# pudnax/voidin

Measured on AMD Instinct MI355X. Metric: M instances culled+compacted/sec, higher is better.
Workload: dtype f32; 1 GPU; configs[2]: 10M synthetic AABB instances, cull + prefix-sum compaction (BASELINE.md §3 distribution, model.rs camera); instances_per_gpu=10000000, instances_total=10000000, n_meshes=16, distribution=baseline, parallelism=single GPU

## Files before the change

### voidin_amd/csrc/cull.hip

```cpp
#include "vd_common.hpp"

#include <math.h>

namespace {

constexpr int kWave = 64;
constexpr int kBlock = 256;
constexpr int kWavesPerBlock = kBlock / kWave;
constexpr int kInstBytes = 144;
constexpr int kSlabBytes = kWave * kInstBytes;
constexpr int kChunksPerLane = kSlabBytes / (kWave * 16);



typedef unsigned int u32x4 __attribute__((ext_vector_type(4)));

struct CullCamera {
    float view[16];
    float frustum[4];
    float znear, zfar;
};

struct MeshRec { float mnx, mny, mnz; unsigned index_count; float mxx, mxy, mxz; unsigned base_index; int vertex_offset; };

// ... 561 lines not shown
    const float d = -c[2];
    const float dn = d - r;
    if (!(dn > znear)) return false;
    const float rr = r * r, dd = d * d, rd = r * d;
    const float tx = sqrtf((c[0] * c[0] + dd) - rr), ty = sqrtf((c[1] * c[1] + dd) - rr);
    const float dxm = d * tx + c[0] * r, dxp = d * tx - c[0] * r, dym = d * ty + c[1] * r, dyp = d * ty - c[1] * r;
    if (!(dxm > 0.0f && dxp > 0.0f && dym > 0.0f && dyp > 0.0f)) return false;
    const float sx0 = (c[0] * tx - rd) / dxm, sx1 = (c[0] * tx + rd) / dxp;
    const float sy0 = (c[1] * ty - rd) / dym, sy1 = (c[1] * ty + rd) / dyp;
    const float nxa = P.p00 * sx0 - P.p20, nxb = P.p00 * sx1 - P.p20, nya = P.p11 * sy0 - P.p21, nyb = P.p11 * sy1 - P.p21;
    const float nx_lo = fminf(nxa, nxb), nx_hi = fmaxf(nxa, nxb), ny_lo = fminf(nya, nyb), ny_hi = fmaxf(nya, nyb);
    const float W = (float)hz.width, H = (float)hz.height;
    const float u0 = (nx_lo * 0.5f + 0.5f) * W - 0.5f, u1 = (nx_hi * 0.5f + 0.5f) * W + 0.5f;
    const float v0 = (0.5f - ny_hi * 0.5f) * H - 0.5f, v1 = (0.5f - ny_lo * 0.5f) * H + 0.5f;
    if (!(u1 >= 0.0f && v1 >= 0.0f && u0 < W && v0 < H)) return false;
    const unsigned x0 = (unsigned)floorf(fmaxf(u0, 0.0f)), x1 = (unsigned)floorf(fminf(u1, W - 1.0f));
    const unsigned y0 = (unsigned)floorf(fmaxf(v0, 0.0f)), y1 = (unsigned)floorf(fminf(v1, H - 1.0f));
    const unsigned span = max(x1 - x0, y1 - y0);
    const unsigned lvl = min(span ? 32u - (unsigned)__clz((int)span) : 0u, hz.n_levels - 1u);
    const float* t = hz.base + hz.off[lvl];
    const unsigned lw = ((hz.width - 1u) >> lvl) + 1u;
    const unsigned ax = x0 >> lvl, bx = x1 >> lvl, ay = y0 >> lvl, by = y1 >> lvl;
    const float h0 = fminf(t[(size_t)ay * lw + ax], t[(size_t)ay * lw + bx]);
    const float h1 = fminf(t[(size_t)by * lw + ax], t[(size_t)by * lw + bx]);
    const float hmin = fminf(h0, h1);
    const float depth = (P.p32 - P.p22 * dn) / dn;
    return depth < hmin;
}

template <typename IdT, bool HIZ, bool PREV>
__global__ __launch_bounds__(kBlock, 3) void cull_mask_occ_kernel(CullCamera cam, OccProj proj, HizView hz, const VdMeshInfo* __restrict__ meshes,
                                                                   unsigned n_mesh, const VdInstance* __restrict__ inst, unsigned n_inst,
                                                                   vd_u64* __restrict__ mask, const vd_u64* prev, vd_u64* visible_out,
                                                                   IdT* __restrict__ ids_out, unsigned* __restrict__ tile_count,
                                                                   unsigned n_tiles) {
    extern __shared__ __attribute__((aligned(16))) char smem[];
    const unsigned lane = threadIdx.x & 63u, wave = threadIdx.x >> 6;
    constexpr int kIdBytes = TileIds<IdT>::kBytes;
    char* slab = smem + wave * (kSlabBytes + kIdBytes);
    IdT* s_ids = reinterpret_cast<IdT*>(slab + kSlabBytes);
    const unsigned waves_total = gridDim.x * kWavesPerBlock;
    const size_t n_words = ((size_t)n_inst + 63) / 64;
    auto valid_at = [&](size_t f) -> unsigned { return f < n_inst ? (unsigned)min((size_t)64, (size_t)n_inst - f) : 0u; };
    u32x4 regs[kChunksPerLane];
    for (unsigned t = blockIdx.x * kWavesPerBlock + wave; t < n_tiles; t += waves_total) {
        const size_t tile_first = (size_t)t * (kWave * kMaskRounds);
        const size_t w0 = (size_t)t * kMaskRounds;
        const bool my_slot = lane < (unsigned)kMaskRounds && w0 + lane < n_words;
        slab_fill<true>(inst, tile_first, valid_at(tile_first), lane, regs);
        unsigned p_lo = 0u, p_hi = 0u;
        if (PREV && my_slot) { const vd_u64 p = prev[w0 + lane]; p_lo = (unsigned)p; p_hi = (unsigned)(p >> 32); }
        TileIds<IdT> tile_ids;
        tile_ids.load(ids_out, tile_first, n_inst, lane);
        vd_u64 list_word = 0, vis_word = 0;
#pragma unroll 1
        for (int r = 0; r < kMaskRounds; ++r) {
            const size_t first = tile_first + (size_t)r * kWave;
            const unsigned n_valid = valid_at(first);
            slab_store(slab, lane, regs);
            if (r + 1 < kMaskRounds) slab_fill<true>(inst, first + kWave, valid_at(first + kWave), lane, regs);
            vd_wave_lds_sync();
            const LaneInst li = slab_read(slab, lane);
            vd_wave_lds_sync();
            const unsigned mid = min(li.mesh, n_mesh - 1u);
            const MeshRec m = load_mesh(meshes, mid);
            const ViewCentre vc = view_centre(cam.view, m, li.T0, li.T1, li.T2, li.T3);
            bool keep = lane < n_valid && frustum_visible(cam, m, vc);
            if (HIZ) {
                if (__ballot(keep) != 0ull) {
                    if (keep) keep = !sphere_occluded(proj, cam.znear, hz, m, vc);
                }
            }
            vd_u64 b = __ballot(keep);
            if (PREV) {
                const vd_u64 p = (vd_u64)(unsigned)__builtin_amdgcn_readlane((int)p_lo, r) |
                                 ((vd_u64)(unsigned)__builtin_amdgcn_readlane((int)p_hi, r) << 32);
                if (HIZ) { if (lane == (unsigned)r) vis_word = b; b &= ~p; }
                else b &= p;
            }
            if (lane == (unsigned)r) list_word = b;
            s_ids[r * kWave + lane] = (IdT)mid;
        }
        vd_wave_lds_sync();
        if (my_slot) {
            mask[w0 + lane] = list_word;
            if (HIZ && PREV) visible_out[w0 + lane] = vis_word;
        }
        unsigned survivors = (unsigned)__popcll(list_word);
#pragma unroll
        for (int off = kMaskRounds / 2; off > 0; off >>= 1) survivors += __shfl_xor(survivors, off);
        if (lane == 0u) tile_count[t] = survivors;
        tile_ids.flush(ids_out, s_ids, tile_first, n_inst, lane);
        vd_wave_lds_sync();
    }
}

constexpr int kExpandGroup = 4;
constexpr int kExpandWords = 32;
constexpr int kChunkWords = kWavesPerBlock * kExpandWords;

constexpr int kScanBlock = 1024;
struct ScanState { unsigned done, epoch, pad[2]; };
__global__ __launch_bounds__(kScanBlock) void mask_scan_kernel(const vd_u64* __restrict__ mask, unsigned n_words, unsigned n_chunks,
                                                           vd_u64* chunk_entry, ScanState* state,
                                                           unsigned* __restrict__ out_count) {
    constexpr int kScanWaves = kScanBlock / kWave;
    __shared__ unsigned s_last, s_wave_sum[kScanWaves];
    const unsigned lane = threadIdx.x & 63u, wave = threadIdx.x >> 6;
    const unsigned ep = __hip_atomic_load(&state->epoch, VD_RLX_AGENT);
    const vd_u64 tag = (vd_u64)ep << 32;
    for (unsigned c = blockIdx.x * kScanWaves + wave; c < n_chunks; c += gridDim.x * kScanWaves) {
        const unsigned w = c * kChunkWords + lane;
        unsigned v = (w < n_words ? (unsigned)__popcll(mask[w]) : 0u) + (w + 64u < n_words ? (unsigned)__popcll(mask[w + 64u]) : 0u);
#pragma unroll
        for (int off = 32; off > 0; off >>= 1) v += __shfl_xor(v, off);
        if (lane == 0) __hip_atomic_store(&chunk_entry[c], tag | v, VD_RLX_AGENT);
    }
    __builtin_amdgcn_s_waitcnt(0);
    __syncthreads();
    if (threadIdx.x == 0) s_last = __hip_atomic_fetch_add(&state->done, 1u, VD_RLX_AGENT) == gridDim.x - 1u;
    __syncthreads();
    if (!s_last) return;
    const unsigned per = (n_chunks + kScanBlock - 1) / kScanBlock;
    const unsigned begin = min(threadIdx.x * per, n_chunks), end = min(begin + per, n_chunks);
    bool stuck = false;
    auto entry = [&](unsigned c) -> unsigned {
        vd_u64 e = __hip_atomic_load(&chunk_entry[c], VD_RLX_AGENT);
        unsigned spins = 0;
        while ((e >> 32) != (vd_u64)ep) {
            if (++spins > (1u << 22)) { stuck = true; return 0u; }
            __builtin_amdgcn_s_sleep(1);
            e = __hip_atomic_load(&chunk_entry[c], VD_RLX_AGENT);
        }
        return (unsigned)e;
    };
    unsigned sum = 0;
    for (unsigned c = begin; c < end; ++c) sum += entry(c);
    const bool any_stuck = __syncthreads_or(stuck ? 1 : 0) != 0;
    unsigned incl = sum;
#pragma unroll
    for (int off = 1; off < kWave; off <<= 1) {
        const unsigned t = __shfl_up(incl, off);
        if (lane >= (unsigned)off) incl += t;
    }
    if (lane == kWave - 1u) s_wave_sum[wave] = incl;
    __syncthreads();
    unsigned run = incl - sum;
    for (unsigned w = 0; w < wave; ++w) run += s_wave_sum[w];
    for (unsigned c = begin; c < end; ++c) {
        if (any_stuck) { chunk_entry[c] = tag | 0xffffffffu; continue; }
        const unsigned v = entry(c);
        chunk_entry[c] = tag | run;
        run += v;
    }
    if (threadIdx.x == kScanBlock - 1u) {
        *out_count = any_stuck ? 0xffffffffu : run;
        __hip_atomic_store(&state->done, 0u, VD_RLX_AGENT);
        __hip_atomic_store(&state->epoch, ep + 1u, VD_RLX_AGENT);
    }
}

constexpr int kChunkTiles = kChunkWords / kMaskRounds;

__device__ __forceinline__ unsigned tile_prefix_partial(const unsigned* __restrict__ tile_count, unsigned n_before) {
    constexpr unsigned kBatch = 4;
    unsigned sum = 0;
    for (unsigned i0 = threadIdx.x * 4u; i0 < n_before; i0 += kBatch * kBlock * 4u) {
        u32x4 v[kBatch];
#pragma unroll
        for (unsigned k = 0; k < kBatch; ++k) {
            const unsigned i = i0 + k * kBlock * 4u;
            v[k] = *reinterpret_cast<const u32x4*>(tile_count + (i < n_before ? i : i0));
        }
#pragma unroll
        for (unsigned k = 0; k < kBatch; ++k) {
            const unsigned i = i0 + k * kBlock * 4u;
            sum += (i < n_before ? v[k].x : 0u) + (i + 1u < n_before ? v[k].y : 0u) + (i + 2u < n_before ? v[k].z : 0u) +
                   (i + 3u < n_before ? v[k].w : 0u);
        }
    }
#pragma unroll
    for (int off = 32; off > 0; off >>= 1) sum += __shfl_xor(sum, off);
    return sum;
}

template <typename IdT, bool TAB, bool TILES>
__global__ __launch_bounds__(kBlock) void expand_mask_kernel(const vd_u64* __restrict__ mask, unsigned n_words, unsigned wps,
                                                             unsigned shard_size, unsigned n_total, unsigned first_instance,
                                                             const IdT* __restrict__ mesh_ids,
                                                             const VdMeshInfo* __restrict__ meshes, unsigned n_mesh,
                                                             VdDrawIndexedIndirect* __restrict__ out,
                                                             const vd_u64* __restrict__ chunk_entry,
                                                             const unsigned* __restrict__ tile_count, unsigned* __restrict__ out_count) {
    constexpr int kGroups = kExpandWords / kExpandGroup;
    __shared__ unsigned s_prefix[kWavesPerBlock];
    constexpr unsigned kTab = TAB ? 512 : 1;
    __shared__ unsigned s_tab[kTab][3];
    constexpr int kStageBytes = kExpandGroup * 1280 + 32;
    __shared__ __attribute__((aligned(16))) char s_stage[kWavesPerBlock][kStageBytes];
    const unsigned lane = threadIdx.x & 63u, wave = threadIdx.x >> 6;
    const unsigned chunk = blockIdx.x;
    const unsigned cw0 = chunk * kChunkWords;
    const unsigned w0 = __builtin_amdgcn_readfirstlane(cw0 + wave * kExpandWords);
    unsigned base = 0;
    if (TILES) {
        const unsigned part = tile_prefix_partial(tile_count, chunk * kChunkTiles);
        if (lane == 0) s_prefix[wave] = part;
    } else {
        base = (unsigned)chunk_entry[chunk];
        if (base == 0xffffffffu) return;
    }
    unsigned before = 0;
    if (lane < wave * kExpandWords && cw0 + lane < n_words) before = (unsigned)__popcll(mask[cw0 + lane]);
    if (lane + 64u < wave * kExpandWords && cw0 + 64u + lane < n_words) before += (unsigned)__popcll(mask[cw0 + 64u + lane]);
    vd_u64 my_word = 0;
    if (lane < (unsigned)kExpandWords && w0 + lane < n_words) my_word = mask[w0 + lane];
    auto group_first = [&](unsigned wg, unsigned (&f)[kExpandGroup]) {
        unsigned shard = wg / wps, r = wg - shard * wps;
#pragma unroll
        for (int q = 0; q < kExpandGroup; ++q) {
            f[q] = shard * shard_size + 64u * r;
            if (++r >= wps) { r = 0u; ++shard; }
        }
    };
    unsigned ids[kExpandWords];
#pragma unroll
    for (int g = 0; g < kGroups; ++g) {
        const unsigned wg = w0 + g * kExpandGroup;
        unsigned f[kExpandGroup];
        group_first(wg, f);
#pragma unroll
        for (int q = 0; q < kExpandGroup; ++q) {
            const unsigned idx = f[q] + lane;
            ids[g * kExpandGroup + q] = (wg + q < n_words && idx < n_total) ? (unsigned)mesh_ids[idx] : 0u;
        }
    }
    if (TAB)
        for (unsigned i = threadIdx.x; i < n_mesh; i += kBlock) {
            s_tab[i][0] = meshes[i].index_count; s_tab[i][1] = meshes[i].base_index; s_tab[i][2] = (unsigned)meshes[i].vertex_offset;
        }
#pragma unroll
    for (int off = 32; off > 0; off >>= 1) before += __shfl_xor(before, off);
    base += before;
    __syncthreads();
    if (TILES) {
#pragma unroll
        for (int w = 0; w < kWavesPerBlock; ++w) base += s_prefix[w];
        if (chunk == gridDim.x - 1u && wave == kWavesPerBlock - 1u) {
            unsigned mine = (unsigned)__popcll(my_word);
#pragma unroll
            for (int off = 32; off > 0; off >>= 1) mine += __shfl_xor(mine, off);
            if (lane == 0) *out_count = base + mine;
        }
    }
    char* stage = s_stage[wave];
#pragma unroll
    for (int g = 0; g < kGroups; ++g) {
        const unsigned wg = w0 + g * kExpandGroup;
        vd_u64 m[kExpandGroup];
        unsigned cnt = 0;
#pragma unroll
        for (int q = 0; q < kExpandGroup; ++q) {
            const int k = g * kExpandGroup + q;
            const unsigned lo = __shfl((unsigned)my_word, k), hi = __shfl((unsigned)(my_word >> 32), k);
            m[q] = ((vd_u64)hi << 32) | lo;
            cnt += (unsigned)__popcll(m[q]);
        }
        if (cnt == 0u) continue;
        char* gbase = reinterpret_cast<char*>(out + base);
        const unsigned shift = (unsigned)(reinterpret_cast<uintptr_t>(gbase) & 15u);
        unsigned run = 0;
        unsigned first[kExpandGroup];
        group_first(wg, first);
#pragma unroll
        for (int q = 0; q < kExpandGroup; ++q) {
            unsigned mid = ids[g * kExpandGroup + q];
            if ((m[q] >> lane) & 1ull) {
                mid = min(mid, n_mesh - 1u);
                unsigned* o = reinterpret_cast<unsigned*>(stage + shift + 20u * (run + vd_mbcnt(m[q])));
                if (TAB) { o[0] = s_tab[mid][0]; o[2] = s_tab[mid][1]; o[3] = s_tab[mid][2]; }
                else { o[0] = meshes[mid].index_count; o[2] = meshes[mid].base_index; o[3] = (unsigned)meshes[mid].vertex_offset; }
                o[1] = 1u;
                o[4] = first_instance + first[q] + lane;
            }
            run += (unsigned)__popcll(m[q]);
        }
        vd_wave_lds_sync();
        const unsigned total = shift + 20u * cnt;
        char* g16 = gbase - shift;
        for (unsigned b0 = lane * 16u; b0 < total; b0 += kWave * 16u) {
            if (b0 >= shift && b0 + 16u <= total) {
                *reinterpret_cast<u32x4*>(g16 + b0) = *reinterpret_cast<const u32x4*>(stage + b0);
            } else {
                const unsigned lo_b = b0 > shift ? b0 : shift, hi_b = b0 + 16u < total ? b0 + 16u : total;
                for (unsigned b = lo_b; b < hi_b; b += 4u)
                    *reinterpret_cast<unsigned*>(g16 + b) = *reinterpret_cast<const unsigned*>(stage + b);
            }
        }
        vd_wave_lds_sync();
        base += cnt;
    }
}

template <bool DIRECT, bool TILES>
__global__ __launch_bounds__(kBlock) void expand_mask_u8_kernel(const vd_u64* __restrict__ mask, unsigned n_words, unsigned wps,
                                                                unsigned shard_size, unsigned n_total, unsigned first_instance,
                                                                const unsigned char* __restrict__ mesh_ids,
                                                                const VdMeshInfo* __restrict__ meshes, unsigned n_mesh,
                                                                VdDrawIndexedIndirect* __restrict__ out,
                                                                const vd_u64* __restrict__ chunk_entry,
                                                                const unsigned* __restrict__ tile_count, unsigned* __restrict__ out_count) {
    constexpr int kGroups = kExpandWords / kExpandGroup;
    __shared__ unsigned s_prefix[kWavesPerBlock];
    __shared__ __attribute__((aligned(16))) unsigned s_tab[256][4];
    constexpr int kStageBytes = DIRECT ? 16 : kExpandGroup * 1280 + 32;
    __shared__ __attribute__((aligned(16))) char s_stage[kWavesPerBlock][kStageBytes];
    const unsigned lane = threadIdx.x & 63u;
    const unsigned wave = __builtin_amdgcn_readfirstlane(threadIdx.x >> 6);
    const unsigned chunk = blockIdx.x;
    const unsigned cw0 = chunk * kChunkWords;
    const unsigned w0 = cw0 + wave * kExpandWords;
    unsigned base = 0;
    if (TILES) {
        const unsigned part = tile_prefix_partial(tile_count, chunk * kChunkTiles);
        if (lane == 0) s_prefix[wave] = part;
    } else {
        base = (unsigned)chunk_entry[chunk];
        if (base == 0xffffffffu) return;
    }
    unsigned before = 0;
    if (lane < wave * kExpandWords && cw0 + lane < n_words) before = (unsigned)__popcll(mask[cw0 + lane]);
    if (lane + 64u < wave * kExpandWords && cw0 + 64u + lane < n_words) before += (unsigned)__popcll(mask[cw0 + 64u + lane]);
    vd_u64 my_word = 0;
    if (lane < (unsigned)kExpandWords && w0 + lane < n_words) my_word = mask[w0 + lane];
    unsigned ids[kGroups];
    {
        const unsigned wl = w0 + (lane >> 4);
        unsigned shard = wl / wps, r = wl - shard * wps;
#pragma unroll
        for (int g = 0; g < kGroups; ++g) {
            const unsigned i0 = shard * shard_size + 64u * r + 4u * (lane & 15u);
            ids[g] = (wl + g * kExpandGroup < n_words && i0 < n_total) ? *reinterpret_cast<const unsigned*>(mesh_ids + i0) : 0u;
            r += kExpandGroup;
            if (r >= wps) { r -= wps; ++shard; }
        }
    }
    unsigned s_shard = w0 / wps, s_r = w0 - s_shard * wps;
    unsigned word_first = s_shard * shard_size + 64u * s_r;
    constexpr unsigned PF = DIRECT ? 0u : 32u;
    unsigned pf = 0;
    if (PF > 0) {
        const unsigned pw = (chunk + 8u * PF) * kChunkWords + (threadIdx.x >> 1);
        if (pw < n_words) {
            const unsigned ps = pw / wps;
            const unsigned pi = ps * shard_size + 64u * (pw - ps * wps) + 32u * (threadIdx.x & 1u);
            if (pi + 32u <= n_total) {
                const u32x4 a = *reinterpret_cast<const u32x4*>(mesh_ids + pi), b = *reinterpret_cast<const u32x4*>(mesh_ids + pi + 16u);
                pf = a.x ^ a.w ^ b.x ^ b.w;
            }
            if ((threadIdx.x & 1u) == 0u) pf ^= (unsigned)mask[pw];
        }
    }
    if (threadIdx.x < n_mesh) {
        const VdMeshInfo mi = meshes[threadIdx.x];
        s_tab[threadIdx.x][0] = mi.index_count; s_tab[threadIdx.x][1] = 1u;
        s_tab[threadIdx.x][2] = mi.base_index;  s_tab[threadIdx.x][3] = (unsigned)mi.vertex_offset;
    }
#pragma unroll
    for (int off = 32; off > 0; off >>= 1) before += __shfl_xor(before, off);
    base = __builtin_amdgcn_readfirstlane(base + before);
    __syncthreads();
    if (TILES) {
#pragma unroll
        for (int w = 0; w < kWavesPerBlock; ++w) base += s_prefix[w];
        base = __builtin_amdgcn_readfirstlane(base);
        if (chunk == gridDim.x - 1u && wave == kWavesPerBlock - 1u) {
            unsigned mine = (unsigned)__popcll(my_word);
#pragma unroll
            for (int off = 32; off > 0; off >>= 1) mine += __shfl_xor(mine, off);
            if (lane == 0) *out_count = base + mine;
        }
    }
    const unsigned max_mid = n_mesh - 1u;
    const unsigned inst_lane = first_instance + lane;
    const unsigned id_shift = 8u * (lane & 3u);
    char* stage = s_stage[wave];
#pragma unroll
    for (int g = 0; g < kGroups; ++g) {
        vd_u64 m[kExpandGroup];
        unsigned cnt = 0;
#pragma unroll
        for (int q = 0; q < kExpandGroup; ++q) {
            const int k = g * kExpandGroup + q;
            const unsigned lo = __builtin_amdgcn_readlane((unsigned)my_word, k), hi = __builtin_amdgcn_readlane((unsigned)(my_word >> 32), k);
            m[q] = ((vd_u64)hi << 32) | lo;
            cnt += (unsigned)__popcll(m[q]);
        }
        unsigned wf[kExpandGroup];
#pragma unroll
        for (int q = 0; q < kExpandGroup; ++q) {
            wf[q] = word_first;
            if (++s_r >= wps) { s_r = 0u; ++s_shard; }
            word_first = s_shard * shard_size + 64u * s_r;
        }
        if (cnt == 0u) continue;
        if (DIRECT) {
            unsigned run = base;
#pragma unroll
            for (int q = 0; q < kExpandGroup; ++q) {
                const unsigned v = (unsigned)__shfl((int)ids[g], q * 16 + (int)(lane >> 2));
                const unsigned mid = min((v >> id_shift) & 0xffu, max_mid);
                if (__builtin_amdgcn_inverse_ballot_w64(m[q])) {
                    unsigned* o = reinterpret_cast<unsigned*>(out + (run + vd_mbcnt(m[q])));
                    typedef u32x4 __attribute__((aligned(4))) u32x4_a4;
                    *reinterpret_cast<u32x4_a4*>(o) = *reinterpret_cast<const u32x4*>(s_tab[mid]);
                    o[4] = inst_lane + wf[q];
                }
                run += (unsigned)__popcll(m[q]);
            }
        } else {
            char* gbase = reinterpret_cast<char*>(out + base);
            const unsigned shift = (unsigned)(reinterpret_cast<uintptr_t>(gbase) & 15u);
            unsigned run = 0;
#pragma unroll
            for (int q = 0; q < kExpandGroup; ++q) {
                const unsigned v = (unsigned)__shfl((int)ids[g], q * 16 + (int)(lane >> 2));
                const unsigned mid = min((v >> id_shift) & 0xffu, max_mid);
                if (__builtin_amdgcn_inverse_ballot_w64(m[q])) {
                    unsigned* o = reinterpret_cast<unsigned*>(stage + shift + 20u * (run + vd_mbcnt(m[q])));
                    const u32x4 c = *reinterpret_cast<const u32x4*>(s_tab[mid]);
                    o[0] = c.x; o[1] = c.y; o[2] = c.z; o[3] = c.w;
                    o[4] = inst_lane + wf[q];
                }
                run += (unsigned)__popcll(m[q]);
            }
            vd_wave_lds_sync();
            const unsigned total = shift + 20u * cnt;
            char* g16 = gbase - shift;
            for (unsigned b0 = lane * 16u; b0 < total; b0 += kWave * 16u) {
                if (b0 >= shift && b0 + 16u <= total) {
                    *reinterpret_cast<u32x4*>(g16 + b0) = *reinterpret_cast<const u32x4*>(stage + b0);
                } else {
                    const unsigned lo_b = b0 > shift ? b0 : shift, hi_b = b0 + 16u < total ? b0 + 16u : total;
                    for (unsigned b = lo_b; b < hi_b; b += 4u)
                        *reinterpret_cast<unsigned*>(g16 + b) = *reinterpret_cast<const unsigned*>(stage + b);
                }
            }
            vd_wave_lds_sync();
        }
        base += cnt;
    }
    if (PF > 0 && pf == 0x9e3779b9u && n_mesh == 0u) out[0].instance_count = pf;
}

template <typename IdT>
__global__ __launch_bounds__(kBlock) void emit_from_mask_kernel(const vd_u64* __restrict__ mask, const IdT* __restrict__ mesh_ids,
                                                               const VdMeshInfo* __restrict__ meshes, unsigned n_mesh,
                                                               unsigned n_inst, unsigned first_instance,
                                                               VdDrawIndexedIndirect* __restrict__ out) {
    constexpr unsigned kTab = 512;
    __shared__ __attribute__((aligned(16))) unsigned s_tab[kTab][4];
    const bool tab = n_mesh <= kTab;
    if (tab)
        for (unsigned i = threadIdx.x; i < n_mesh; i += kBlock) {
            s_tab[i][0] = meshes[i].index_count; s_tab[i][1] = 0u;
            s_tab[i][2] = meshes[i].base_index;  s_tab[i][3] = (unsigned)meshes[i].vertex_offset;
        }
    __syncthreads();
    const unsigned n_quads = (n_inst + 3u) / 4u;
    for (unsigned q = blockIdx.x * kBlock + threadIdx.x; q < n_quads; q += gridDim.x * kBlock) {
        const unsigned i0 = q * 4u;
        const unsigned bits = (unsigned)(mask[i0 >> 6] >> (i0 & 63u)) & 15u;
        unsigned mid[4];
#pragma unroll
        for (int k = 0; k < 4; ++k) mid[k] = i0 + k < n_inst ? min((unsigned)mesh_ids[i0 + k], n_mesh - 1u) : 0u;
        unsigned w[20];
#pragma unroll
        for (int k = 0; k < 4; ++k) {
            u32x4 c;
            if (tab) c = *reinterpret_cast<const u32x4*>(s_tab[mid[k]]);
            else { c.x = meshes[mid[k]].index_count; c.z = meshes[mid[k]].base_index; c.w = (unsigned)meshes[mid[k]].vertex_offset; }
            w[5 * k] = c.x; w[5 * k + 1] = (bits >> k) & 1u; w[5 * k + 2] = c.z; w[5 * k + 3] = c.w; w[5 * k + 4] = first_instance + i0 + k;
        }
        unsigned* o = reinterpret_cast<unsigned*>(out + i0);
        if (i0 + 4u <= n_inst) {
#pragma unroll
            for (int k = 0; k < 5; ++k) {
                u32x4 v; v.x = w[4 * k]; v.y = w[4 * k + 1]; v.z = w[4 * k + 2]; v.w = w[4 * k + 3];
                *reinterpret_cast<u32x4*>(o + 4 * k) = v;
            }
        } else {
            for (unsigned k = 0; k < 5u * (n_inst - i0); ++k) o[k] = w[k];
        }
    }
}

__global__ __launch_bounds__(kBlock) void emit_all_u8_kernel(const vd_u64* __restrict__ mask, unsigned n_words, unsigned n_inst,
                                                             unsigned first_instance, const unsigned char* __restrict__ mesh_ids,
                                                             const VdMeshInfo* __restrict__ meshes, unsigned n_mesh,
                                                             VdDrawIndexedIndirect* __restrict__ out) {
    constexpr int kGroups = kExpandWords / kExpandGroup;
    __shared__ __attribute__((aligned(16))) unsigned s_tab[256][4];
    const unsigned lane = threadIdx.x & 63u;
    const unsigned wave = __builtin_amdgcn_readfirstlane(threadIdx.x >> 6);
    const unsigned w0 = (blockIdx.x * kWavesPerBlock + wave) * kExpandWords;
    vd_u64 my_word = 0;
    if (lane < (unsigned)kExpandWords && w0 + lane < n_words) my_word = mask[w0 + lane];
    unsigned ids[kGroups];
#pragma unroll
    for (int g = 0; g < kGroups; ++g) {
        const unsigned i0 = 64u * (w0 + g * kExpandGroup + (lane >> 4)) + 4u * (lane & 15u);
        ids[g] = i0 < n_inst ? *reinterpret_cast<const unsigned*>(mesh_ids + i0) : 0u;
    }
    if (threadIdx.x < n_mesh) {
        const VdMeshInfo mi = meshes[threadIdx.x];
        s_tab[threadIdx.x][0] = mi.index_count; s_tab[threadIdx.x][1] = 0u;
        s_tab[threadIdx.x][2] = mi.base_index;  s_tab[threadIdx.x][3] = (unsigned)mi.vertex_offset;
    }
    __syncthreads();
    const unsigned max_mid = n_mesh - 1u;
    const unsigned id_shift = 8u * (lane & 3u);
#pragma unroll
    for (int g = 0; g < kGroups; ++g) {
#pragma unroll
        for (int q = 0; q < kExpandGroup; ++q) {
            const int k = g * kExpandGroup + q;
            const unsigned lo = __builtin_amdgcn_readlane((unsigned)my_word, k), hi = __builtin_amdgcn_readlane((unsigned)(my_word >> 32), k);
            const vd_u64 m = ((vd_u64)hi << 32) | lo;
            const unsigned v = (unsigned)__shfl((int)ids[g], q * 16 + (int)(lane >> 2));
            const unsigned mid = min((v >> id_shift) & 0xffu, max_mid);
            const unsigned i = 64u * (w0 + (unsigned)k) + lane;
            if (i < n_inst) {
                u32x4 c = *reinterpret_cast<const u32x4*>(s_tab[mid]);
                c.y = (unsigned)(m >> lane) & 1u;
                unsigned* o = reinterpret_cast<unsigned*>(out + i);
                typedef u32x4 __attribute__((aligned(4))) u32x4_a4;
                *reinterpret_cast<u32x4_a4*>(o) = c;
                o[4] = first_instance + i;
            }
        }
    }
}

__global__ __launch_bounds__(kBlock) void mask_to_indices_kernel(const vd_u64* __restrict__ mask, unsigned n_words, unsigned first_instance,
                                                                 unsigned* __restrict__ out, const vd_u64* __restrict__ chunk_entry) {
    const unsigned lane = threadIdx.x & 63u;
    const unsigned wave = __builtin_amdgcn_readfirstlane(threadIdx.x >> 6);
    const unsigned cw0 = blockIdx.x * kChunkWords;
    const unsigned w0 = cw0 + wave * kExpandWords;
    unsigned base = (unsigned)chunk_entry[blockIdx.x];
    if (base == 0xffffffffu) return;
    unsigned before = 0;
    if (lane < wave * kExpandWords && cw0 + lane < n_words) before = (unsigned)__popcll(mask[cw0 + lane]);
    if (lane + 64u < wave * kExpandWords && cw0 + 64u + lane < n_words) before += (unsigned)__popcll(mask[cw0 + 64u + lane]);
    vd_u64 my_word = 0;
    if (lane < (unsigned)kExpandWords && w0 + lane < n_words) my_word = mask[w0 + lane];
#pragma unroll
    for (int off = 32; off > 0; off >>= 1) before += __shfl_xor(before, off);
    base = __builtin_amdgcn_readfirstlane(base + before);
    const unsigned inst_lane = first_instance + 64u * w0 + lane;
#pragma unroll
    for (int k = 0; k < kExpandWords; ++k) {
        const unsigned lo = __builtin_amdgcn_readlane((unsigned)my_word, k), hi = __builtin_amdgcn_readlane((unsigned)(my_word >> 32), k);
        const vd_u64 m = ((vd_u64)hi << 32) | lo;
        if (__builtin_amdgcn_inverse_ballot_w64(m)) out[base + vd_mbcnt(m)] = inst_lane + 64u * (unsigned)k;
        base += (unsigned)__popcll(m);
    }
}

template <typename IdT>
__global__ __launch_bounds__(kBlock) void indices_to_draws_kernel(const unsigned* __restrict__ indices, unsigned n_indices,
                                                                  const IdT* __restrict__ mesh_ids, unsigned n_total,
                                                                  const VdMeshInfo* __restrict__ meshes, unsigned n_mesh,
                                                                  VdDrawIndexedIndirect* __restrict__ out) {
    constexpr unsigned kTab = 512;
    __shared__ __attribute__((aligned(16))) unsigned s_tab[kTab][4];
    const bool tab = n_mesh <= kTab;
    if (tab)
        for (unsigned i = threadIdx.x; i < n_mesh; i += kBlock) {
            s_tab[i][0] = meshes[i].index_count; s_tab[i][1] = 1u;
            s_tab[i][2] = meshes[i].base_index;  s_tab[i][3] = (unsigned)meshes[i].vertex_offset;
        }
    __syncthreads();
    for (unsigned k = blockIdx.x * kBlock + threadIdx.x; k < n_indices; k += gridDim.x * kBlock) {
        const unsigned i = indices[k];
        const unsigned mid = min((unsigned)mesh_ids[min(i, n_total - 1u)], n_mesh - 1u);
        u32x4 c;
        if (tab) c = *reinterpret_cast<const u32x4*>(s_tab[mid]);
        else { c.x = meshes[mid].index_count; c.y = 1u; c.z = meshes[mid].base_index; c.w = (unsigned)meshes[mid].vertex_offset; }
        unsigned* o = reinterpret_cast<unsigned*>(out + k);
        typedef u32x4 __attribute__((aligned(4))) u32x4_a4;
        *reinterpret_cast<u32x4_a4*>(o) = c;
        o[4] = i;
    }
}

static int launch_mask_scan(VdCtx* ctx, const vd_u64* d_mask, unsigned n_words, unsigned* d_out_count, vd_u64** out_entries) {
    const unsigned n_chunks = (n_words + kChunkWords - 1) / kChunkWords;
    const size_t need = sizeof(ScanState) + (size_t)n_chunks * 8;
    if (need > ctx->expand_state_bytes || !ctx->expand_state) {
        int rc = vd_ensure(ctx, &ctx->expand_state, &ctx->expand_state_bytes, need);
        if (rc) return rc;
        VD_HIP_CHECK(ctx, hipMemsetAsync(ctx->expand_state, 0, ctx->expand_state_bytes, ctx->stream));
        VD_HIP_CHECK(ctx, hipMemsetD32Async(reinterpret_cast<hipDeviceptr_t>(reinterpret_cast<char*>(ctx->expand_state) + offsetof(ScanState, epoch)), 1, 1, ctx->stream));
    }
    ScanState* state = reinterpret_cast<ScanState*>(ctx->expand_state);
    vd_u64* entries = reinterpret_cast<vd_u64*>(reinterpret_cast<char*>(ctx->expand_state) + sizeof(ScanState));
    unsigned sblocks = (n_chunks + 15u) / 16u;
    if (sblocks > (unsigned)ctx->num_cus * 2u) sblocks = (unsigned)ctx->num_cus * 2u;
    hipLaunchKernelGGL(mask_scan_kernel, dim3(sblocks), dim3(kScanBlock), 0, ctx->stream, d_mask, n_words, n_chunks, entries, state,
                       d_out_count);
    *out_entries = entries;
    return VD_OK;
}

static int launch_expand(VdCtx* ctx, const vd_u64* d_mask, unsigned n_words, unsigned wps, unsigned shard_size,
                         unsigned n_total, unsigned first_instance, const void* d_ids, unsigned id_bytes,
                         const VdMeshInfo* d_meshes, unsigned n_mesh, VdDrawIndexedIndirect* d_out, unsigned* d_out_count,
                         const unsigned* d_tile_count = nullptr) {
    const unsigned n_chunks = (n_words + kChunkWords - 1) / kChunkWords;
    vd_u64* offsets = nullptr;
    if (!d_tile_count) {
        int rc_scan = launch_mask_scan(ctx, d_mask, n_words, d_out_count, &offsets);
        if (rc_scan) return rc_scan;
    }
    const bool one_shard = wps >= n_words;
    const bool tab = n_mesh <= 512u;
    const bool fast = id_bytes == 1u && n_mesh <= 256u && (one_shard || (shard_size % 4u == 0u && wps >= (unsigned)kExpandGroup)) &&
                      (reinterpret_cast<uintptr_t>(d_ids) & 3u) == 0u;
    if (fast) {
#define VD_EXPAND_U8(D, T)                                                                                                  \
        hipLaunchKernelGGL((expand_mask_u8_kernel<D, T>), dim3(n_chunks), dim3(kBlock), 0, ctx->stream, d_mask, n_words, wps, \
                           shard_size, n_total, first_instance, reinterpret_cast<const unsigned char*>(d_ids), d_meshes,      \
                           n_mesh, d_out, offsets, d_tile_count, d_out_count)
        const bool direct = n_total <= (12u << 20);
        if (d_tile_count) { if (direct) VD_EXPAND_U8(true, true); else VD_EXPAND_U8(false, true); }
        else { if (direct) VD_EXPAND_U8(true, false); else VD_EXPAND_U8(false, false); }
#undef VD_EXPAND_U8
        return VD_OK;
    }
#define VD_EXPAND_T(IdT, T, S)                                                                                             \
    hipLaunchKernelGGL((expand_mask_kernel<IdT, T, S>), dim3(n_chunks), dim3(kBlock), 0, ctx->stream, d_mask, n_words, wps, \
                       shard_size, n_total, first_instance, reinterpret_cast<const IdT*>(d_ids), d_meshes, n_mesh, d_out,    \
                       offsets, d_tile_count, d_out_count)
#define VD_EXPAND(IdT, T) do { if (d_tile_count) VD_EXPAND_T(IdT, T, true); else VD_EXPAND_T(IdT, T, false); } while (0)
    if (id_bytes == 1u) { if (tab) VD_EXPAND(unsigned char, true); else VD_EXPAND(unsigned char, false); }
    else if (id_bytes == 2u) { if (tab) VD_EXPAND(unsigned short, true); else VD_EXPAND(unsigned short, false); }
    else { if (tab) VD_EXPAND(unsigned, true); else VD_EXPAND(unsigned, false); }
#undef VD_EXPAND
#undef VD_EXPAND_T
    return VD_OK;
}

__global__ __launch_bounds__(kBlock) void pad_tail_kernel(VdDrawIndexedIndirect* __restrict__ out,
                                                          const unsigned* __restrict__ count, unsigned n) {
    const unsigned c = *count;
    const size_t begin = (c > n ? (size_t)0 : (size_t)c) * 5u, end = (size_t)n * 5u;
    unsigned* o = reinterpret_cast<unsigned*>(out);
    if (begin >= end) return;
    const size_t gid = (size_t)blockIdx.x * kBlock + threadIdx.x, gsz = (size_t)gridDim.x * kBlock;
    const size_t mis = (reinterpret_cast<uintptr_t>(o + begin) >> 2) & 3u;
    const size_t head = min(end - begin, (4u - mis) & 3u);
    const size_t quads = (end - begin - head) >> 2;
    const size_t tail_first = begin + head + quads * 4u;
    if (gid < head) o[begin + gid] = 0u;
    if (gid < end - tail_first) o[tail_first + gid] = 0u;
    u32x4* q = reinterpret_cast<u32x4*>(o + begin + head);
    const u32x4 z = {0u, 0u, 0u, 0u};
    for (size_t i = gid; i < quads; i += gsz) __builtin_nontemporal_store(z, q + i);
}

constexpr int kCompactPerThread = 8;
constexpr int kCompactTile = kBlock * kCompactPerThread;

__global__ __launch_bounds__(kBlock) void compact_draws_kernel(const VdDrawIndexedIndirect* __restrict__ in, unsigned n,
                                                               VdDrawIndexedIndirect* __restrict__ out,
                                                               unsigned* __restrict__ out_count, vd_u64* tile_state,
                                                               vd_u64* ticket_counter, unsigned n_tiles, unsigned* fault_host) {
    __shared__ unsigned s_ticket, s_epoch, s_wave_total[kWavesPerBlock], s_tile_excl;
    const unsigned lane = threadIdx.x & 63u, wave = threadIdx.x >> 6;
    if (threadIdx.x == 0) s_ticket = vd_take_ticket(ticket_counter, n_tiles, &s_epoch);
    __syncthreads();
    const unsigned tile = s_ticket, epoch = s_epoch;
    if (tile >= n_tiles) return;
    if (tile == 0u && threadIdx.x == 0) { __hip_atomic_store(out_count, VD_SCAN_STUCK, VD_RLX_AGENT); __threadfence(); }
    const size_t wave_first = (size_t)tile * kCompactTile + (size_t)wave * (kWave * kCompactPerThread);
    unsigned long long masks[kCompactPerThread];
    unsigned wave_total = 0;
    const unsigned* in32 = reinterpret_cast<const unsigned*>(in);
#pragma unroll
    for (int r = 0; r < kCompactPerThread; ++r) {
        const size_t i = wave_first + (size_t)r * kWave + lane;
        const bool keep = i < n && in32[i * 5u + 1u] == 1u;
        masks[r] = __ballot(keep);
        wave_total += (unsigned)__popcll(masks[r]);
    }
    if (lane == 0) s_wave_total[wave] = wave_total;
    __syncthreads();
    if (wave == 0) {
        unsigned tile_total = 0;
#pragma unroll
        for (int w = 0; w < kWavesPerBlock; ++w) tile_total += s_wave_total[w];
        const unsigned excl = vd_lookback(tile_state, epoch, tile, tile_total);
        if (lane == 0) {
            s_tile_excl = excl;
            if (tile == n_tiles - 1u) *out_count = vd_scan_final_count(tile_state, epoch, excl, tile_total, fault_host);
        }
    }
    __syncthreads();
    unsigned base = s_tile_excl;
    if (base == VD_SCAN_STUCK) return;
    for (unsigned w = 0; w < wave; ++w) base += s_wave_total[w];
    unsigned* out32 = reinterpret_cast<unsigned*>(out);
#pragma unroll
    for (int r = 0; r < kCompactPerThread; ++r) {
        const unsigned long long mask = masks[r];
        if ((mask >> lane) & 1ull) {
            const size_t i = wave_first + (size_t)r * kWave + lane;
            const size_t d = (size_t)(base + vd_mbcnt(mask)) * 5u;
#pragma unroll
            for (int k = 0; k < 5; ++k) out32[d + k] = in32[i * 5u + k];
        }
        base += (unsigned)__popcll(mask);
    }
}

struct RotZ { float c_pos, s_pos, c_neg, s_neg; };
template <int SRC> __device__ __forceinline__ float quad_bcast(float v) {
    return __int_as_float(__builtin_amdgcn_mov_dpp(__float_as_int(v), SRC * 0x55, 0xf, 0xf, true));
}
__global__ __launch_bounds__(256) void compute_update_kernel(const unsigned* __restrict__ indices, unsigned n_indices,
                                                             VdInstance* __restrict__ inst, unsigned n_inst, RotZ rz, int fix_inverse) {
    const unsigned t = blockIdx.x * 256u + threadIdx.x, k = t >> 2, col = t & 3u;
    const unsigned idx = k < n_indices ? indices[k] : 0xffffffffu;
    const bool live = idx < n_inst;
    float4* t4 = reinterpret_cast<float4*>(inst[live ? idx : 0u].transform);
    float4 v = make_float4(0.0f, 0.0f, 0.0f, 0.0f);
    if (live) v = t4[col];
    const float t14 = quad_bcast<3>(v.z);
    const bool pos = t14 > -15.0f;
    const float c = pos ? rz.c_pos : rz.c_neg, s = pos ? rz.s_pos : rz.s_neg;
    float4 o;
    o.x = ((c * v.x + -s * v.y) + 0.0f * v.z) + 0.0f * v.w;
    o.y = ((s * v.x + c * v.y) + 0.0f * v.z) + 0.0f * v.w;
    o.z = ((0.0f * v.x + 0.0f * v.y) + 1.0f * v.z) + 0.0f * v.w;
    o.w = ((0.0f * v.x + 0.0f * v.y) + 0.0f * v.z) + 1.0f * v.w;
    if (live) t4[col] = o;
    if (fix_inverse) {
        float4* i4 = reinterpret_cast<float4*>(inst[live ? idx : 0u].inv_transform);
        float4 w = make_float4(0.0f, 0.0f, 0.0f, 0.0f);
        if (live) w = i4[col];
        const float4 I0 = make_float4(quad_bcast<0>(w.x), quad_bcast<0>(w.y), quad_bcast<0>(w.z), quad_bcast<0>(w.w));
        const float4 I1 = make_float4(quad_bcast<1>(w.x), quad_bcast<1>(w.y), quad_bcast<1>(w.z), quad_bcast<1>(w.w));
        const float4 I2 = make_float4(quad_bcast<2>(w.x), quad_bcast<2>(w.y), quad_bcast<2>(w.z), quad_bcast<2>(w.w));
        const float4 I3 = make_float4(quad_bcast<3>(w.x), quad_bcast<3>(w.y), quad_bcast<3>(w.z), quad_bcast<3>(w.w));
        const float b0 = col == 0u ? c : (col == 1u ? s : 0.0f);
        const float b1 = col == 0u ? -s : (col == 1u ? c : 0.0f);
        const float b2 = col == 2u ? 1.0f : 0.0f, b3 = col == 3u ? 1.0f : 0.0f;
        float4 r;
        r.x = ((I0.x * b0 + I1.x * b1) + I2.x * b2) + I3.x * b3;
        r.y = ((I0.y * b0 + I1.y * b1) + I2.y * b2) + I3.y * b3;
        r.z = ((I0.z * b0 + I1.z * b1) + I2.z * b2) + I3.z * b3;
        r.w = ((I0.w * b0 + I1.w * b1) + I2.w * b2) + I3.w * b3;
        if (live) i4[col] = r;
    }
}

CullCamera make_cam(const VdCameraUniform* c) {
    CullCamera k;
    memcpy(k.view, c->view, sizeof(k.view));
    memcpy(k.frustum, c->frustum, sizeof(k.frustum));
    k.znear = c->znear;
    k.zfar = c->zfar;
    return k;
}

}

extern "C" {

int vd_cull_emit_dev(VdCtx* ctx, const VdCameraUniform* camera, const VdMeshInfo* d_meshes, uint32_t n_mesh,
                     const VdInstance* d_instances, uint32_t n_inst, VdDrawIndexedIndirect* d_out) {
    VdDeviceGuard vd_guard_(ctx);
    return vd_cull_emit_shard_dev(ctx, camera, d_meshes, n_mesh, d_instances, n_inst, 0u, d_out);
}

static int launch_mask_pass(VdCtx* ctx, const VdCameraUniform* camera, const VdMeshInfo* d_meshes, uint32_t n_mesh,
                            const VdInstance* d_instances, uint32_t n_inst, vd_u64** out_mask, void** out_ids, unsigned* out_id_bytes,
                            unsigned** out_tile_count) {
    const unsigned n_words = (n_inst + 63u) / 64u;
    const unsigned id_bytes = n_mesh <= 256u ? 1u : (n_mesh <= 65536u ? 2u : 4u);
    const unsigned n_mt = (n_inst + kWave * kMaskRounds - 1) / (kWave * kMaskRounds);
    const size_t ids_off = ((size_t)n_words * 8 + 255) & ~(size_t)255;
    const size_t counts_off = (ids_off + (size_t)n_inst * id_bytes + 15) & ~(size_t)15;
    const size_t need = counts_off + (((size_t)n_mt + 3) & ~(size_t)3) * 4 + 512;
    int rc = vd_ensure(ctx, &ctx->scratch, &ctx->scratch_bytes, need);
    if (rc) return rc;
    vd_u64* d_mask = reinterpret_cast<vd_u64*>(ctx->scratch);
    void* d_ids = reinterpret_cast<char*>(ctx->scratch) + ids_off;
    unsigned* d_counts = reinterpret_cast<unsigned*>(reinterpret_cast<char*>(ctx->scratch) + counts_off);
    vd_time_begin(ctx);
    unsigned mb = (n_mt + kWavesPerBlock - 1) / kWavesPerBlock;
    if (mb > (unsigned)ctx->num_cus * 3u) mb = (unsigned)ctx->num_cus * 3u;
#define VD_SPLIT(IdT)                                                                                              \
    hipLaunchKernelGGL(cull_mask_tiled_kernel<IdT>, dim3(mb), dim3(kBlock),                                        \
                       kWavesPerBlock * (kSlabBytes + kMaskRounds * kWave * (int)sizeof(IdT)),                     \
                       ctx->stream, make_cam(camera), d_meshes, n_mesh, d_instances, n_inst, d_mask,               \
                       reinterpret_cast<IdT*>(d_ids), d_counts, n_mt)
    if (id_bytes == 1u) VD_SPLIT(unsigned char);
    else if (id_bytes == 2u) VD_SPLIT(unsigned short);
    else VD_SPLIT(unsigned);
#undef VD_SPLIT
    vd_time_mid(ctx);
    *out_mask = d_mask; *out_ids = d_ids; *out_id_bytes = id_bytes; *out_tile_count = d_counts;
    return VD_OK;
}

int vd_cull_emit_shard_dev(VdCtx* ctx, const VdCameraUniform* camera, const VdMeshInfo* d_meshes, uint32_t n_mesh,
                           const VdInstance* d_instances, uint32_t n_inst, uint32_t first_instance,
                           VdDrawIndexedIndirect* d_out) {
    VdDeviceGuard vd_guard_(ctx);
    if (!ctx) return VD_ERR_INVALID_ARG;
    if (!camera || !d_meshes || n_mesh == 0) VD_FAIL(ctx, VD_ERR_INVALID_ARG, "vd_cull_emit: null camera/meshes or n_mesh == 0");
    if (n_inst == 0) return VD_OK;
    if (!d_instances || !d_out) VD_FAIL(ctx, VD_ERR_INVALID_ARG, "vd_cull_emit: null instances/out");
    if (ctx->option(VD_OPT_CULL_VARIANT, 0) <= 0 && n_inst >= ctx->split_min) {
        vd_u64* d_mask; void* d_ids; unsigned id_bytes; unsigned* d_tile_count;
        int rc = launch_mask_pass(ctx, camera, d_meshes, n_mesh, d_instances, n_inst, &d_mask, &d_ids, &id_bytes, &d_tile_count);
        if (rc) return rc;
        const unsigned quads = (n_inst + 3u) / 4u;
        unsigned eb = (quads + kBlock - 1) / kBlock;
        if (eb > (unsigned)ctx->num_cus * 16u) eb = (unsigned)ctx->num_cus * 16u;
#define VD_EMIT(IdT) hipLaunchKernelGGL(emit_from_mask_kernel<IdT>, dim3(eb), dim3(kBlock), 0, ctx->stream, d_mask,               \
                                        reinterpret_cast<const IdT*>(d_ids), d_meshes, n_mesh, n_inst, first_instance, d_out)
        if (id_bytes == 1u) {
            const unsigned n_words = (n_inst + 63u) / 64u;
            hipLaunchKernelGGL(emit_all_u8_kernel, dim3((n_words + kChunkWords - 1) / kChunkWords), dim3(kBlock), 0, ctx->stream, d_mask,
                               n_words, n_inst, first_instance, reinterpret_cast<const unsigned char*>(d_ids), d_meshes, n_mesh, d_out);
        } else if (id_bytes == 2u) VD_EMIT(unsigned short); else VD_EMIT(unsigned);
#undef VD_EMIT
        vd_time_end(ctx);
        VD_HIP_CHECK(ctx, hipGetLastError());
        return VD_OK;
    }
    const unsigned n_wave_tiles = (n_inst + kWave - 1) / kWave;
    unsigned blocks = (n_wave_tiles + kWavesPerBlock - 1) / kWavesPerBlock;
    const unsigned cap = (unsigned)ctx->num_cus * 4u;
    if (blocks > cap) blocks = cap;
    vd_time_begin(ctx);
    hipLaunchKernelGGL(emit_draws_kernel, dim3(blocks), dim3(kBlock), kWavesPerBlock * kSlabBytes, ctx->stream,
                       make_cam(camera), d_meshes, n_mesh, d_instances, n_inst, d_out, n_wave_tiles, first_instance);
    vd_time_end(ctx);
    VD_HIP_CHECK(ctx, hipGetLastError());
    return VD_OK;
}

int vd_cull_compact_dev(VdCtx* ctx, const VdCameraUniform* camera, const VdMeshInfo* d_meshes, uint32_t n_mesh,
                        const VdInstance* d_instances, uint32_t n_inst, VdDrawIndexedIndirect* d_out,
                        uint32_t* d_out_count, int pad_tail) {
    VdDeviceGuard vd_guard_(ctx);
    return vd_cull_compact_shard_dev(ctx, camera, d_meshes, n_mesh, d_instances, n_inst, 0u, d_out, d_out_count, pad_tail);
}

int vd_cull_compact_shard_dev(VdCtx* ctx, const VdCameraUniform* camera, const VdMeshInfo* d_meshes, uint32_t n_mesh,
                              const VdInstance* d_instances, uint32_t n_inst, uint32_t first_instance,
                              VdDrawIndexedIndirect* d_out, uint32_t* d_out_count, int pad_tail) {
    VdDeviceGuard vd_guard_(ctx);
    if (!ctx) return VD_ERR_INVALID_ARG;
    if (!camera || !d_meshes || n_mesh == 0 || !d_out_count)
        VD_FAIL(ctx, VD_ERR_INVALID_ARG, "vd_cull_compact: null camera/meshes/count or n_mesh == 0");
    if (n_inst == 0) {
        VD_HIP_CHECK(ctx, hipMemsetAsync(d_out_count, 0, 4, ctx->stream));
        return VD_OK;
    }
    if (!d_instances || !d_out) VD_FAIL(ctx, VD_ERR_INVALID_ARG, "vd_cull_compact: null instances/out");
    const int variant = (int)ctx->option(VD_OPT_CULL_VARIANT, 0);
    vd_u64* ticket; vd_u64* states;
    int rc = vd_scan_check_fault(ctx);
    if (rc) return rc;
    if (variant <= 0 && n_inst >= ctx->split_min) {
        vd_u64* d_mask; void* d_ids; unsigned id_bytes; unsigned* d_tile_count;
        rc = launch_mask_pass(ctx, camera, d_meshes, n_mesh, d_instances, n_inst, &d_mask, &d_ids, &id_bytes, &d_tile_count);
        if (rc) return rc;
        const unsigned n_words = (n_inst + 63u) / 64u;
        rc = launch_expand(ctx, d_mask, n_words, n_words, n_inst, n_inst, first_instance, d_ids, id_bytes, d_meshes, n_mesh,
                           d_out, d_out_count, d_tile_count);
        if (rc) return rc;
        vd_time_end(ctx);
        if (pad_tail) {
            unsigned pblocks = (unsigned)ctx->num_cus * 4u;
            hipLaunchKernelGGL(pad_tail_kernel, dim3(pblocks), dim3(kBlock), 0, ctx->stream, d_out, d_out_count, n_inst);
        }
        VD_HIP_CHECK(ctx, hipGetLastError());
        return VD_OK;
    }
#define VD_LAUNCH_COMPACT(R)                                                                                     \
    do {                                                                                                         \
        const unsigned n_tiles = (n_inst + kBlock * (R) - 1) / (kBlock * (R));                                   \
        rc = vd_scan_scratch(ctx, n_tiles, &ticket, &states, true);                                              \
        if (rc) return rc;                                                                                       \
        hipLaunchKernelGGL((cull_compact_kernel<R>), dim3(n_tiles), dim3(kBlock), (compact_lds_bytes<R>()),      \
                           ctx->stream, make_cam(camera), d_meshes, n_mesh, d_instances, n_inst, d_out,          \
                           d_out_count, states, ticket, n_tiles, first_instance, vd_scan_fault_word(ctx));       \
    } while (0)
    const int rounds = variant > 0 ? variant : (n_inst >= (4u << 20) ? 32 : (n_inst >= (5u << 18) ? 16 : (n_inst >= 600000u ? 8 : (n_inst >= 192000u ? 4 : (n_inst >= 48000u ? 2 : 1)))));
    switch (rounds) {
        case 1: VD_LAUNCH_COMPACT(1); break;
        case 2: VD_LAUNCH_COMPACT(2); break;
        case 4: VD_LAUNCH_COMPACT(4); break;
        case 8: VD_LAUNCH_COMPACT(8); break;
        case 16: VD_LAUNCH_COMPACT(16); break;
        default: VD_LAUNCH_COMPACT(32); break;
    }
#undef VD_LAUNCH_COMPACT
    vd_time_end(ctx);
    if (pad_tail) {
        unsigned blocks = (unsigned)ctx->num_cus * 4u;
        hipLaunchKernelGGL(pad_tail_kernel, dim3(blocks), dim3(kBlock), 0, ctx->stream, d_out, d_out_count, n_inst);
    }
    VD_HIP_CHECK(ctx, hipGetLastError());
    return VD_OK;
}

int vd_cull_compact_views_dev(VdCtx* ctx, const VdCameraUniform* cameras, uint32_t n_views, const VdMeshInfo* d_meshes, uint32_t n_mesh,
                              const VdInstance* d_instances, uint32_t n_inst, VdDrawIndexedIndirect* d_out, uint64_t out_stride,
                              uint32_t* d_out_counts, int pad_tail) {
    VdDeviceGuard vd_guard_(ctx);
    if (!ctx) return VD_ERR_INVALID_ARG;
    if (!cameras || !d_meshes || n_mesh == 0 || !d_out_counts)
        VD_FAIL(ctx, VD_ERR_INVALID_ARG, "vd_cull_compact_views: null cameras/meshes/counts or n_mesh == 0");
    if (n_views == 0 || n_views > (uint32_t)VD_MAX_VIEWS) VD_FAIL(ctx, VD_ERR_INVALID_ARG, "vd_cull_compact_views: n_views must be 1..VD_MAX_VIEWS");
    if (out_stride < n_inst) VD_FAIL(ctx, VD_ERR_INVALID_ARG, "vd_cull_compact_views: out_stride < n_inst");
    if (n_inst == 0) {
        VD_HIP_CHECK(ctx, hipMemsetAsync(d_out_counts, 0, 4 * (size_t)n_views, ctx->stream));
        return VD_OK;
    }
    if (!d_instances || !d_out) VD_FAIL(ctx, VD_ERR_INVALID_ARG, "vd_cull_compact_views: null instances/out");
    if (n_views == 1) return vd_cull_compact_dev(ctx, cameras, d_meshes, n_mesh, d_instances, n_inst, d_out, d_out_counts, pad_tail);
    const unsigned n_words = (n_inst + 63u) / 64u;
    const unsigned id_bytes = n_mesh <= 256u ? 1u : (n_mesh <= 65536u ? 2u : 4u);
// ... 475 lines not shown
```

Before: 39680 M instances/s.

## Stage compacted draw commands in LDS and flush full 128-byte aligned lines

Replaces the direct scattered 20-byte global stores (used for inputs of 12M instances or fewer, which covers the 10M config) with LDS staging for all sizes. Each wave carries partial output across groups and writes only whole 128-byte aligned segments with 16-byte vector stores, keeping the unaligned tail in LDS for the next group. The goal is fewer partial-line writes and better write coalescing to the output buffer. The cost is extra LDS traffic and wave-level syncs, plus a larger staging buffer that can lower occupancy.

```diff
diff --git a/voidin_amd/csrc/cull.hip b/voidin_amd/csrc/cull.hip
--- a/voidin_amd/csrc/cull.hip
+++ b/voidin_amd/csrc/cull.hip
@@ -887,7 +887,7 @@
     }
 }
 
-template <bool DIRECT, bool TILES>
+template <bool PREFETCH, bool TILES>
 __global__ __launch_bounds__(kBlock) void expand_mask_u8_kernel(const vd_u64* __restrict__ mask, unsigned n_words, unsigned wps,
                                                                 unsigned shard_size, unsigned n_total, unsigned first_instance,
                                                                 const unsigned char* __restrict__ mesh_ids,
@@ -898,7 +898,8 @@
     constexpr int kGroups = kExpandWords / kExpandGroup;
     __shared__ unsigned s_prefix[kWavesPerBlock];
     __shared__ __attribute__((aligned(16))) unsigned s_tab[256][4];
-    constexpr int kStageBytes = DIRECT ? 16 : kExpandGroup * 1280 + 32;
+    constexpr unsigned P = 128;
+    constexpr int kStageBytes = kExpandGroup * 1280 + (int)P;
     __shared__ __attribute__((aligned(16))) char s_stage[kWavesPerBlock][kStageBytes];
     const unsigned lane = threadIdx.x & 63u;
     const unsigned wave = __builtin_amdgcn_readfirstlane(threadIdx.x >> 6);
@@ -932,7 +933,7 @@
     }
     unsigned s_shard = w0 / wps, s_r = w0 - s_shard * wps;
     unsigned word_first = s_shard * shard_size + 64u * s_r;
-    constexpr unsigned PF = DIRECT ? 0u : 32u;
+    constexpr unsigned PF = PREFETCH ? 32u : 0u;
     unsigned pf = 0;
     if (PF > 0) {
         const unsigned pw = (chunk + 8u * PF) * kChunkWords + (threadIdx.x >> 1);
@@ -970,6 +971,19 @@
     const unsigned inst_lane = first_instance + lane;
     const unsigned id_shift = 8u * (lane & 3u);
     char* stage = s_stage[wave];
+    unsigned pos = (unsigned)(reinterpret_cast<uintptr_t>(out + base) & (P - 1u)), lo = pos;
+    char* gorg = reinterpret_cast<char*>(out + base) - pos;
+    auto flush = [&](unsigned from, unsigned to, unsigned hp) {
+        unsigned he = (from + hp - 1u) & ~(hp - 1u);
+        he = he < to ? he : to;
+        if (from + 4u * lane < he) *reinterpret_cast<unsigned*>(gorg + from + 4u * lane) = *reinterpret_cast<const unsigned*>(stage + from + 4u * lane);
+        const unsigned be = he + ((to - he) & ~15u);
+        for (unsigned b = he + 16u * lane; b < be; b += kWave * 16u) {
+            const u32x4 v = *reinterpret_cast<const u32x4*>(stage + b);
+            *reinterpret_cast<u32x4*>(gorg + b) = v;
+        }
+        if (be + 4u * lane < to) *reinterpret_cast<unsigned*>(gorg + be + 4u * lane) = *reinterpret_cast<const unsigned*>(stage + be + 4u * lane);
+    };
 #pragma unroll
     for (int g = 0; g < kGroups; ++g) {
         vd_u64 m[kExpandGroup];
@@ -989,52 +1003,34 @@
             word_first = s_shard * shard_size + 64u * s_r;
         }
         if (cnt == 0u) continue;
-        if (DIRECT) {
-            unsigned run = base;
-#pragma unroll
-            for (int q = 0; q < kExpandGroup; ++q) {
-                const unsigned v = (unsigned)__shfl((int)ids[g], q * 16 + (int)(lane >> 2));
-                const unsigned mid = min((v >> id_shift) & 0xffu, max_mid);
-                if (__builtin_amdgcn_inverse_ballot_w64(m[q])) {
-                    unsigned* o = reinterpret_cast<unsigned*>(out + (run + vd_mbcnt(m[q])));
-                    typedef u32x4 __attribute__((aligned(4))) u32x4_a4;
-                    *reinterpret_cast<u32x4_a4*>(o) = *reinterpret_cast<const u32x4*>(s_tab[mid]);
-                    o[4] = inst_lane + wf[q];
-                }
-                run += (unsigned)__popcll(m[q]);
+        unsigned run = 0;
+#pragma unroll
+        for (int q = 0; q < kExpandGroup; ++q) {
+            const unsigned v = (unsigned)__shfl((int)ids[g], q * 16 + (int)(lane >> 2));
+            const unsigned mid = min((v >> id_shift) & 0xffu, max_mid);
+            if (__builtin_amdgcn_inverse_ballot_w64(m[q])) {
+                unsigned* o = reinterpret_cast<unsigned*>(stage + pos + 20u * (run + vd_mbcnt(m[q])));
+                const u32x4 c = *reinterpret_cast<const u32x4*>(s_tab[mid]);
+                o[0] = c.x; o[1] = c.y; o[2] = c.z; o[3] = c.w;
+                o[4] = inst_lane + wf[q];
             }
+            run += (unsigned)__popcll(m[q]);
+        }
+        vd_wave_lds_sync();
+        const unsigned end = pos + 20u * cnt, whole = end & ~(P - 1u);
+        if (whole > lo) {
+            flush(lo, whole, P);
+            unsigned carry = 0;
+            if (whole + 4u * lane < end) carry = *reinterpret_cast<const unsigned*>(stage + whole + 4u * lane);
+            if (whole + 4u * lane < end) *reinterpret_cast<unsigned*>(stage + 4u * lane) = carry;
+            gorg += whole; pos = end - whole; lo = 0u;
         } else {
-            char* gbase = reinterpret_cast<char*>(out + base);
-            const unsigned shift = (unsigned)(reinterpret_cast<uintptr_t>(gbase) & 15u);
-            unsigned run = 0;
-#pragma unroll
-            for (int q = 0; q < kExpandGroup; ++q) {
-                const unsigned v = (unsigned)__shfl((int)ids[g], q * 16 + (int)(lane >> 2));
-                const unsigned mid = min((v >> id_shift) & 0xffu, max_mid);
-                if (__builtin_amdgcn_inverse_ballot_w64(m[q])) {
-                    unsigned* o = reinterpret_cast<unsigned*>(stage + shift + 20u * (run + vd_mbcnt(m[q])));
-                    const u32x4 c = *reinterpret_cast<const u32x4*>(s_tab[mid]);
-                    o[0] = c.x; o[1] = c.y; o[2] = c.z; o[3] = c.w;
-                    o[4] = inst_lane + wf[q];
-                }
-                run += (unsigned)__popcll(m[q]);
-            }
-            vd_wave_lds_sync();
-            const unsigned total = shift + 20u * cnt;
-            char* g16 = gbase - shift;
-            for (unsigned b0 = lane * 16u; b0 < total; b0 += kWave * 16u) {
-                if (b0 >= shift && b0 + 16u <= total) {
-                    *reinterpret_cast<u32x4*>(g16 + b0) = *reinterpret_cast<const u32x4*>(stage + b0);
-                } else {
-                    const unsigned lo_b = b0 > shift ? b0 : shift, hi_b = b0 + 16u < total ? b0 + 16u : total;
-                    for (unsigned b = lo_b; b < hi_b; b += 4u)
-                        *reinterpret_cast<unsigned*>(g16 + b) = *reinterpret_cast<const unsigned*>(stage + b);
-                }
-            }
-            vd_wave_lds_sync();
-        }
+            pos = end;
+        }
+        vd_wave_lds_sync();
         base += cnt;
     }
+    if (pos > lo) flush(lo, pos, 16u);
     if (PF > 0 && pf == 0x9e3779b9u && n_mesh == 0u) out[0].instance_count = pf;
 }
 
@@ -1214,13 +1210,13 @@
     const bool fast = id_bytes == 1u && n_mesh <= 256u && (one_shard || (shard_size % 4u == 0u && wps >= (unsigned)kExpandGroup)) &&
                       (reinterpret_cast<uintptr_t>(d_ids) & 3u) == 0u;
     if (fast) {
-#define VD_EXPAND_U8(D, T)                                                                                                  \
-        hipLaunchKernelGGL((expand_mask_u8_kernel<D, T>), dim3(n_chunks), dim3(kBlock), 0, ctx->stream, d_mask, n_words, wps, \
+#define VD_EXPAND_U8(PFETCH, T)                                                                                                  \
+        hipLaunchKernelGGL((expand_mask_u8_kernel<PFETCH, T>), dim3(n_chunks), dim3(kBlock), 0, ctx->stream, d_mask, n_words, wps, \
                            shard_size, n_total, first_instance, reinterpret_cast<const unsigned char*>(d_ids), d_meshes,      \
                            n_mesh, d_out, offsets, d_tile_count, d_out_count)
-        const bool direct = n_total <= (12u << 20);
-        if (d_tile_count) { if (direct) VD_EXPAND_U8(true, true); else VD_EXPAND_U8(false, true); }
-        else { if (direct) VD_EXPAND_U8(true, false); else VD_EXPAND_U8(false, false); }
+        const bool prefetch = n_total > (12u << 20);
+        if (d_tile_count) { if (prefetch) VD_EXPAND_U8(true, true); else VD_EXPAND_U8(false, true); }
+        else { if (prefetch) VD_EXPAND_U8(true, false); else VD_EXPAND_U8(false, false); }
 #undef VD_EXPAND_U8
         return VD_OK;
     }
```

Measured after the change: 40060 M instances/s (median of 6 runs). No clear change (+1.0%).
